# Icelk/strange-attractor-renderer

Measured on AMD Instinct MI355X. Metric: attractor iterations/sec at 1e9 iters, 2048x2048 buffer (poisson-saturne), per-GPU frame, higher is better.
Workload: dtype f64

## Files before the change

strange_attractor_renderer_amd/csrc/sar_iterate.hip:

```cpp
#include "sar_device.hpp"
#include "sar_launch.hpp"

namespace sar {

__global__ void __launch_bounds__(256) k_iterate(const IterArgs a) {
    const uint32_t job = blockIdx.x * blockDim.x + threadIdx.x;
    if (job >= a.n_jobs) return;
    MapParams p = a.p;
#pragma unroll
    for (int k = 0; k < 9; ++k) p.m[k] = vgpr_pin(p.m[k]);
    p.sin_v = vgpr_pin(p.sin_v);
    p.cos_v = vgpr_pin(p.cos_v);
    p.ccx = vgpr_pin(p.ccx);
    p.ccy = vgpr_pin(p.ccy);
    p.ccz = vgpr_pin(p.ccz);
    p.width = vgpr_pin(p.width);
    p.height = vgpr_pin(p.height);
    p.half_height = vgpr_pin(p.half_height);
    p.width_scaled = vgpr_pin(p.width_scaled);
    p.scale_adjusted_mid = vgpr_pin(p.scale_adjusted_mid);

    double x = a.starts[job];
    double y = a.starts[a.n_jobs + job];
    double z = a.starts[2u * a.n_jobs + job];

    if (!a.resume)
        for (int w = 0; w < 1000; ++w) next_point(p, x, y, z);

    const uint32_t n = (uint32_t)a.iters;
    const uint32_t lo_base = 0xFFFFFFFFu - job * n;
    const uint32_t C = a.ckpt_stride;
    const size_t cs = a.n_jobs;

    uint32_t t = 0;
    double* ck = a.ckpt + job;
    bool ended = false;
    while (t < n && !ended) {
        ck[0] = x;
        ck[cs] = y;
        ck[2 * cs] = z;
        ck += 3 * cs;
        const uint32_t tend = (n - t > C) ? t + C : n;
        for (; t < tend; ++t) {
            next_point(p, x, y, z);
            if (x != x) {
                __hip_atomic_fetch_add(a.scratch_count, n - t, __ATOMIC_RELAXED, __HIP_MEMORY_SCOPE_AGENT);
                ended = true;
                break;
            }
            double sx, sy, sz;
            screen_space(p, x, y, z, sx, sy, sz);
            const double ax = sx + p.ccx;
            const double az = sz + p.ccy;
            const double x2 = ax * p.cos_v + az * p.sin_v;
            const double z2 = ax * p.sin_v - az * p.cos_v;
            const double fi = (p.scale_adjusted_mid - x2) * p.width_scaled;
            const double fj = p.half_height - (sy + p.ccz) * p.width_scaled;
            if (fi >= p.width || fj >= p.height || fi < 0. || fj < 0.) continue;
            const uint32_t i = (fi == fi) ? (uint32_t)fi : 0u;
            const uint32_t j = (fj == fj) ? (uint32_t)fj : 0u;
            const uint32_t idx = j * a.width + i;
            __hip_atomic_fetch_add(a.scratch_count + idx, 1u, __ATOMIC_RELAXED, __HIP_MEMORY_SCOPE_AGENT);
            float zf = (float)z2;
            if (zf > -1.0f) {
                zf = zf + 0.0f;
                const unsigned long long k =
                    ((unsigned long long)f32_sortable(zf) << 32) | (unsigned long long)(lo_base - t);
                __hip_atomic_fetch_max(a.scratch_key + idx, k, __ATOMIC_RELAXED, __HIP_MEMORY_SCOPE_AGENT);
            }
        }
    }
    if (a.state_out) {
        a.state_out[job] = x;
        a.state_out[a.n_jobs + job] = y;
        a.state_out[2u * a.n_jobs + job] = z;
    }
}


template <bool DEPTH, uint32_t U, typename H, uint32_t W = 0>
struct DepthPipe {
    static_assert(W % U == 0, "a park window is whole passes of the depth pipeline");
    static constexpr bool kWide = sizeof(H) == 4;
    H* zhint;
    unsigned long long* key;
    uint32_t lo_base;
    HintQuant hq;
    HintTile ht;
    bool pv[U];
    uint32_t p_idx[U], p_zf[U], p_hint[U], p_q[U], n_sent, n_pass;
    uint32_t p_t[U];
    bool gv[U];
    uint32_t g_idx[U], g_q[U];
    unsigned long long g_mine[U], g_cur[U];
    unsigned long long q_m;
    unsigned long long pvm[U];
    uint32_t q_idx, q_zf, q_t;

    __device__ __forceinline__ uint32_t hint_index(uint32_t idx) const {
        if (kWide) return idx;
        return bfi(ht.mask2, bfi(ht.mask1, idx >> ht.shift1, idx << 3), idx);
    }
    __device__ __forceinline__ void depth_init(H* zhint_, unsigned long long* key_, uint32_t lo_base_, const uint32_t* hint_range_, const HintTile& tile_) {
        ht = tile_;
        zhint = zhint_;
        key = key_;
        lo_base = lo_base_;
        hq = hint_quant(kWide ? nullptr : hint_range_);
        n_sent = n_pass = 0;
#pragma unroll
        for (uint32_t k = 0; k < U; ++k) {
            pv[k] = gv[k] = false;
            p_idx[k] = p_zf[k] = p_hint[k] = p_q[k] = p_t[k] = 0;
            g_idx[k] = g_q[k] = 0;
            g_mine[k] = g_cur[k] = 0;
        }
        q_m = 0ull;
#pragma unroll
        for (uint32_t k = 0; k < U; ++k) pvm[k] = 0ull;
        q_idx = q_zf = q_t = 0;
    }

#ifdef SAR_EXPERIMENT_PROF
    unsigned long long dprof[2] = {0, 0};
#define SAR_DMARK(i, t0) do { asm volatile("s_waitcnt vmcnt(0)" ::: "memory"); const unsigned long long n_ = __builtin_readcyclecounter(); dprof[i] += n_ - t0; t0 = n_; } while (0)
#else
#define SAR_DMARK(i, t0)
#endif
    __device__ __forceinline__ void key_settle(uint32_t k) {
        if (g_mine[k] > g_cur[k]) {
            atomicMax(key + g_idx[k], g_mine[k]);
            ++n_sent;
        }
        const uint32_t seen = (uint32_t)(g_cur[k] >> 32);
        uint32_t learnt;
        if (kWide) {
            const float mine = __uint_as_float(g_q[k]), theirs = sortable_f32(seen);
            learnt = (seen && theirs > mine) ? __float_as_uint(theirs) : g_q[k];
        } else {
            const uint32_t qs = seen ? depth_q16(sortable_f32(seen), hq) : 0u;
            learnt = qs > g_q[k] ? qs : g_q[k];
        }
        zhint[hint_index(g_idx[k])] = (H)learnt;
    }
    __device__ __forceinline__ void key_request(uint32_t k, uint32_t idx, uint32_t zf, uint32_t q, uint32_t t) {
        ++n_pass;
        const float zc = __uint_as_float(zf) + 0.0f;
        g_idx[k] = idx;
        g_q[k] = kWide ? __float_as_uint(zc) : q;
        g_mine[k] = ((unsigned long long)f32_sortable(zc) << 32) | (unsigned long long)(lo_base - t);
        g_cur[k] = __hip_atomic_load(key + idx, __ATOMIC_RELAXED, __HIP_MEMORY_SCOPE_AGENT);
    }
    __device__ __forceinline__ bool hint_passed(uint32_t k) const {
        if (kWide) return pv[k] && __uint_as_float(p_zf[k]) >= __uint_as_float(p_hint[k]);
        const uint32_t hint = (p_idx[k] & 1u) ? (p_hint[k] >> 16) : (p_hint[k] & 0xFFFFu);
        return pv[k] && p_q[k] >= hint;
    }
    __device__ __forceinline__ void settle_depth(uint32_t k) {
#ifdef SAR_EXPERIMENT_PROF
        unsigned long long t0_ = __builtin_readcyclecounter();
#endif
        if (gv[k]) key_settle(k);
        SAR_DMARK(0, t0_);
        gv[k] = hint_passed(k);
        if (gv[k]) key_request(k, p_idx[k], p_zf[k], p_q[k], p_t[k]);
        SAR_DMARK(1, t0_);
    }

    __device__ __forceinline__ unsigned long long pass_mask(uint32_t k) const {
        if (kWide) return pvm[k] & __builtin_amdgcn_fcmpf(__uint_as_float(p_zf[k]), __uint_as_float(p_hint[k]), 3 );
        const uint32_t hint = (p_idx[k] & 1u) ? (p_hint[k] >> 16) : (p_hint[k] & 0xFFFFu);
        return pvm[k] & lanes_ge(p_q[k], hint);
    }
    __device__ __forceinline__ void park_flush() {
        if (gv[0]) key_settle(0);
        const bool parked = __builtin_amdgcn_inverse_ballot_w64(q_m);
        gv[0] = parked;
        if (parked) key_request(0, q_idx, q_zf, kWide ? 0u : depth_q16(__uint_as_float(q_zf) + 0.0f, hq), q_t);
        q_m = 0ull;
    }
    __device__ __forceinline__ void settle_parked(uint32_t k, bool window) {
        const unsigned long long pm = pass_mask(k);
        if (window || (pm & q_m) != 0ull) park_flush();
        q_m |= pm;
        if (__builtin_amdgcn_inverse_ballot_w64(pm)) {
            q_idx = p_idx[k];
            q_zf = p_zf[k];
            q_t = p_t[k];
            asm volatile("" : "+v"(q_idx), "+v"(q_zf), "+v"(q_t));
        }
    }

    __device__ __forceinline__ bool depth_candidate(uint32_t k, bool inb, uint32_t idx, float zf, uint32_t t) {
        if (!DEPTH) return false;
        if (W) settle_parked(k, k == 0u && (t & (W - 1u)) == 0u);
        else settle_depth(k);
        p_idx[k] = idx;
        p_zf[k] = __float_as_uint(zf);
        p_t[k] = t;
        if (kWide) {
            pv[k] = inb;
            if (W) pvm[k] = wave_ballot(inb);
            return inb;
        }
        const bool cand = inb && zf > -1.0f;
        p_q[k] = depth_q16(zf + 0.0f, hq);
        pv[k] = cand;
        if (W) pvm[k] = wave_ballot(inb) & __builtin_amdgcn_fcmpf(zf, -1.0f, 2 );
        return cand;
    }

    __device__ __forceinline__ void depth_request(uint32_t k, bool cand, uint32_t idx) {
        if (DEPTH) p_hint[k] = *(const uint32_t*)(zhint + (cand ? (kWide ? idx : (hint_index(idx) & ~1u)) : 0u));
    }

    __device__ __forceinline__ void depth_drain(uint32_t lane, unsigned long long* stats) {
        if (!DEPTH) return;
        if (W) {
#pragma unroll
            for (uint32_t k = 0; k < U; ++k) {
                settle_parked(k, false);
                pv[k] = false;
                pvm[k] = 0ull;
            }
            park_flush();
            park_flush();
        } else {
#pragma unroll
            for (uint32_t k = 0; k < U; ++k) {
                settle_depth(k);
                pv[k] = false;
            }
#pragma unroll
            for (uint32_t k = 0; k < U; ++k) settle_depth(k);
        }
        uint32_t tot = n_sent, pas = n_pass;
        for (int off = 32; off > 0; off >>= 1) {
            tot += __shfl_down(tot, off);
            pas += __shfl_down(pas, off);
        }
        if (lane == 0 && tot) atomicAdd(stats + 1, (unsigned long long)tot);
        if (lane == 0 && pas) atomicAdd(stats + 14, (unsigned long long)pas);
    }
};

template <bool DEPTH, uint32_t R, uint32_t U, typename H, uint32_t W = 0>
struct PoolStager : DepthPipe<DEPTH, U, H, W> {
    using DepthPipe<DEPTH, U, H, W>::depth_init;
    using DepthPipe<DEPTH, U, H, W>::depth_candidate;
    using DepthPipe<DEPTH, U, H, W>::depth_request;
    using DepthPipe<DEPTH, U, H, W>::depth_drain;
    static constexpr uint32_t CB = kPoolChunkBytes(R);
    static constexpr uint32_t Q = CB / 16u;
    static constexpr uint32_t P = kPoolSpareOf(R);
    static constexpr uint32_t kFillBits = 7u, kFillMask = 127u;
    uint32_t* ctl;
    uint32_t* ring;
    uint32_t pool0;
    uint32_t lane, n_bins;
    uint4* arena;
    uint32_t cursor;
    uint32_t drained;
    BinMap map;
    uint32_t bin_bits_v;
    bool b_have;
    uint32_t b_bin, b_old, b_local;
#ifdef SAR_EXPERIMENT_PROF
    unsigned long long prof[8] = {0, 0, 0, 0, 0, 0, 0, 0}, prof_last = 0;
    __device__ __forceinline__ void mark(int i) {
        asm volatile("" ::: "memory");
        const unsigned long long now = __builtin_readcyclecounter();
        asm volatile("" ::: "memory");
        prof[i] += now - prof_last;
        prof_last = now;
    }
#define SAR_MARK(i) this->mark(i)
#else
#define SAR_MARK(i)
#endif

    static __device__ __forceinline__ uint32_t lds_addr(const void* p) { return (uint32_t)(uintptr_t)(const __attribute__((address_space(3))) void*)p; }
    static __device__ __forceinline__ char* lds_ptr(uint32_t a) { return (char*)(__attribute__((address_space(3))) char*)(uintptr_t)a; }

    __device__ __forceinline__ void init(char* wbase, uint32_t bins, uint32_t lane_, uint4* arena_, H* zhint_,
                                         unsigned long long* key_, const BinMap& map_, uint32_t lo_base_, const uint32_t* hint_range_, const HintTile& tile_) {
        n_bins = bins;
        lane = lane_;
        char* pool = wbase;
        ctl = (uint32_t*)(wbase + (bins + P) * CB);
        ring = ctl + bins;
        pool0 = lds_addr(pool) + 8u;
        for (uint32_t b = lane; b < bins; b += 64u) {
            ctl[b] = (pool0 + b * CB) << kFillBits;
            *(uint2*)(pool + b * CB) = make_uint2(kNoChunk, R);
        }
        if (lane < P) ring[lane] = pool0 + (bins + lane) * CB;
        arena = arena_;
        cursor = drained = 0;
        depth_init(zhint_, key_, lo_base_, hint_range_, tile_);
        map = map_;
        bin_bits_v = map_.bin_bits;
        asm volatile("" : "+v"(bin_bits_v));
        b_have = false;
        b_bin = b_old = b_local = 0;
    }

    __device__ __forceinline__ void drain_all() {
        constexpr uint32_t G = kChunkLanes(R);
        static_assert(P <= 64u / G, "one pass must cover the ring");
        const uint32_t q = lane % G;
        const uint32_t e = drained + lane / G;
        if ((int32_t)(cursor - e) > 0 && q < Q) {
            const uint32_t rec = ring[e % P];
            const u32x4 v = *(const u32x4*)lds_ptr(rec - 8u + q * 16u);
            __builtin_nontemporal_store(v, (u32x4*)(arena + (size_t)e * kChunkStride(R)) + q);
        }
        drained = cursor;
    }

    __device__ __forceinline__ void swap_round(bool mine, uint32_t rank, uint32_t count, uint32_t bin, uint32_t rec) {
        if (cursor - drained + count > P) drain_all();
        if (mine) {
            const uint32_t chunk = cursor + rank;
            const uint32_t fresh = __hip_atomic_exchange(&ring[chunk % P], rec, __ATOMIC_RELAXED, __HIP_MEMORY_SCOPE_WORKGROUP);
            *(uint2*)lds_ptr(fresh - 8u) = make_uint2(chunk, R);
            __hip_atomic_fetch_add(&ctl[bin], ((fresh - rec) << kFillBits) - R, __ATOMIC_RELAXED, __HIP_MEMORY_SCOPE_WORKGROUP);
        }
        cursor = __builtin_amdgcn_readfirstlane(cursor + count);
    }
    __device__ __forceinline__ void swap_full(bool fl, unsigned long long fb, uint32_t bin, uint32_t rec) {
        const uint32_t rank = __builtin_amdgcn_mbcnt_hi((uint32_t)(fb >> 32), __builtin_amdgcn_mbcnt_lo((uint32_t)fb, 0u));
        const uint32_t nfill = (uint32_t)__popcll(fb);
        if (nfill <= P) {
            swap_round(fl, rank, nfill, bin, rec);
        } else {
            for (uint32_t base = 0; base < nfill; base += P)
                swap_round(fl && rank - base < P, rank - base, nfill - base < P ? nfill - base : P, bin, rec);
        }
    }

    __device__ __forceinline__ void place_visit() {
        uint32_t slot = b_old & kFillMask;
        uint32_t rec = b_old >> kFillBits;
        const bool w0 = b_have && slot < R;
        if (w0) *(unsigned short*)lds_ptr(rec + 2u * slot) = (unsigned short)b_local;
        const unsigned long long fb = lanes_eq(slot, R - 1u) & wave_ballot(b_have);
        const bool fl = b_have && slot == R - 1u;
        if (fb) {
            swap_full(fl, fb, b_bin, rec);
            if (__builtin_expect(lanes_ge(b_have ? slot : 0u, R) != 0ull, 0)) place_overflow(slot, rec);
        }
    }
    __device__ __forceinline__ void place_overflow(uint32_t slot, uint32_t rec) {
        bool over = b_have && slot >= R;
        for (;;) {
            slot -= over ? R : 0u;
            if (over) rec = ctl[b_bin] >> kFillBits;
            const bool w = over && slot < R;
            if (w) *(unsigned short*)lds_ptr(rec + 2u * slot) = (unsigned short)b_local;
            const bool fl = w && slot == R - 1u;
            over = over && slot >= R;
            const unsigned long long fb = wave_ballot(fl);
            if (!fb) break;
            swap_full(fl, fb, b_bin, rec);
            if (!wave_ballot(over)) break;
        }
    }

    __device__ __forceinline__ void step(uint32_t k, bool inb, uint32_t idx, float zf, uint32_t t) {
        __builtin_amdgcn_s_setprio(3);
        place_visit();
        SAR_MARK(2);
        const bool cand = depth_candidate(k, inb, idx, zf, t);
        SAR_MARK(3);
        b_have = inb;
        b_bin = __builtin_amdgcn_ubfe(idx, map.seg_shift, bin_bits_v);
        b_local = bfi(map.low_mask, idx, idx >> map.hi_shift);
        if (inb) b_old = atomicAdd(&ctl[b_bin], 1u);
        depth_request(k, cand, idx);
        __builtin_amdgcn_s_setprio(0);
        SAR_MARK(4);
    }

    __device__ __forceinline__ void finish(uint32_t* heads, uint32_t n_waves, uint32_t wave, unsigned long long* stats) {
        place_visit();
        drain_all();
        depth_drain(lane, stats);
        for (uint32_t b0 = 0; b0 < n_bins; b0 += 64u) {
            const uint32_t b = b0 + lane;
            const uint32_t word = (b < n_bins) ? ctl[b] : (pool0 << kFillBits);
            const uint32_t have = (b < n_bins) ? (word & kFillMask) : 0u;
            const bool flusher = have != 0u;
            const unsigned long long fb = wave_ballot(flusher);
            const uint32_t rec = word >> kFillBits;
            uint32_t head = (b < n_bins) ? *(const uint32_t*)lds_ptr(rec - 8u) : kNoChunk;
            if (flusher) {
                const uint32_t chunk = cursor + __builtin_amdgcn_mbcnt_hi((uint32_t)(fb >> 32),
                                                                          __builtin_amdgcn_mbcnt_lo((uint32_t)fb, 0u));
                *(uint32_t*)lds_ptr(rec - 4u) = have;
                u32x4* dst = (u32x4*)(arena + (size_t)chunk * kChunkStride(R));
#pragma unroll
                for (uint32_t q = 0; q < Q; ++q)
                    __builtin_nontemporal_store(*(const u32x4*)lds_ptr(rec - 8u + q * 16u), dst + q);
                head = chunk;
            }
            cursor += (uint32_t)__popcll(fb);
            if (b < n_bins) heads[(size_t)b * n_waves + wave] = head;
        }
    }
};

constexpr int kWarmupRangeIters = 64;
__device__ __forceinline__ void warmup_body(const WarmArgs& a) {
    const double* __restrict__ starts = a.starts;
    double* __restrict__ warm = a.warm;
    uint32_t* __restrict__ joblist = a.joblist;
    uint32_t* const hint_range = a.hint_range;
    const uint32_t n_jobs = a.n_jobs;
    const uint32_t slot_in = blockIdx.x * blockDim.x + threadIdx.x;
    const uint32_t n_in = a.in_active ? *a.in_active : n_jobs;
    if (blockIdx.x * blockDim.x >= n_in) return;
    const bool valid = slot_in < n_in;
    const uint32_t job = (valid && a.in_joblist) ? a.in_joblist[slot_in] : slot_in;
    const int n_iter = (int)a.n_iter;
    MapParams p = a.p;
    pin_map_params(p);
    double x = 0., y = 0., z = 0.;
    float zlo = __builtin_inff(), zhi = -__builtin_inff();
    if (valid) {
        x = starts[slot_in];
        y = starts[n_jobs + slot_in];
        z = starts[2u * n_jobs + slot_in];
        if (!hint_range) {
            for (int w = 0; w < n_iter; ++w) next_point(p, x, y, z);
        } else {
            const int n_range = n_iter < kWarmupRangeIters ? n_iter : kWarmupRangeIters;
            for (int w = 0; w < n_iter - n_range; ++w) next_point(p, x, y, z);
            for (int w = 0; w < n_range; ++w) {
                bool inb;
                uint32_t idx;
                float zf;
                iterate_once(p, a.width, x, y, z, inb, idx, zf);
                if (inb && zf > -1.0f) {
                    zlo = fminf(zlo, zf);
                    zhi = fmaxf(zhi, zf);
                }
            }
        }
    }
    if (hint_range) {
        for (int off = 32; off > 0; off >>= 1) {
            zlo = fminf(zlo, __shfl_down(zlo, off));
            zhi = fmaxf(zhi, __shfl_down(zhi, off));
        }
        if ((threadIdx.x & 63u) == 0u && zhi >= zlo) {
            atomicMax(hint_range, ~f32_sortable(zlo + 0.0f));
            atomicMax(hint_range + 1, f32_sortable(zhi + 0.0f));
        }
    }
    const bool live = valid && x == x;
    const unsigned long long lm = wave_ballot(live), dm = wave_ballot(valid && !live);
    const uint32_t rank = __builtin_amdgcn_mbcnt_hi((uint32_t)(lm >> 32), __builtin_amdgcn_mbcnt_lo((uint32_t)lm, 0u));
    uint32_t base = 0;
    if ((threadIdx.x & 63u) == 0u) {
        if (lm) base = atomicAdd(a.active, (uint32_t)__popcll(lm));
        if (dm) atomicAdd(a.nan_count, a.iters * (unsigned long long)__popcll(dm));
    }
    base = __builtin_amdgcn_readfirstlane(base);
    if (live) {
        const uint32_t slot = base + rank;
        warm[slot] = x;
        warm[n_jobs + slot] = y;
        warm[2u * n_jobs + slot] = z;
        joblist[slot] = job;
    }
}
__global__ void __launch_bounds__(256) k_warmup(const WarmArgs a) { warmup_body(a); }

__global__ void __launch_bounds__(256) k_warmup_batch(const BatchFrame* frames, uint32_t first_phase) {
    const WarmArgs a = load_frame_args(first_phase ? &frames[blockIdx.z].warm_first : &frames[blockIdx.z].warm);
    warmup_body(a);
}
__global__ void __launch_bounds__(256) k_batch_clear(const BatchFrame* frames) {
    const BatchFrame* f = frames + blockIdx.y;
    uint32_t* const seg = f->seg_any;
    const uint32_t n = f->seg_words;
    for (uint32_t k = blockIdx.x * blockDim.x + threadIdx.x; k < n; k += gridDim.x * blockDim.x) seg[k] = 0u;
    if (blockIdx.x == 0u && threadIdx.x < 4u) f->warm.active[threadIdx.x] = 0u;
    if (blockIdx.x == 0u && threadIdx.x < 4u && f->warm_first.n_iter) f->warm_first.active[threadIdx.x] = 0u;
    if (blockIdx.x == 0u && threadIdx.x < 2u && f->clear_hint_range) f->warm.hint_range[threadIdx.x] = 0u;
}

template <bool DEPTH, uint32_t R, uint32_t U, typename H>
__global__ void __launch_bounds__(256) k_iterate_lean(const BinIterArgs a) {
    extern __shared__ __attribute__((aligned(16))) uint32_t smem[];
    const uint32_t lane = threadIdx.x & 63u;
    const uint32_t slot = blockIdx.x * blockDim.x + threadIdx.x;
    const uint32_t wave = slot >> 6;
    const uint32_t active = *a.active;
    if (a.warm_nan && slot == 0u) {
        const unsigned long long dead = *a.warm_nan;
        if (dead) atomicAdd(a.nan_count, dead);
    }
    if ((slot & ~63u) >= active) {
        for (uint32_t b = lane; b < a.n_bins; b += 64u) a.heads[(size_t)b * a.n_waves + wave] = kNoChunk;
        return;
    }
    bool alive = slot < active;
    const uint32_t job = alive ? a.joblist[slot] : 0u;
    const uint32_t n = (uint32_t)a.it.iters;

    PoolStager<DEPTH, R, U, H> st;
    st.init((char*)smem + (threadIdx.x >> 6) * kPoolWaveLds(a.n_bins, R), a.n_bins, lane,
            (uint4*)a.arena + (size_t)wave * a.chunks_per_wave * kChunkStride(R),
            (H*)a.zhint + (size_t)(xcc_id() & a.hint_copy_mask) * kHintStride(a.it.npix), a.it.scratch_key, a.map, 0xFFFFFFFFu - job * n, a.hint_range, a.tile);

    MapParams p = a.it.p;
    pin_map_params(p);
#pragma unroll
    for (int k = 0; k < 10; ++k) p.cy[k] = vgpr_pin(p.cy[k]);
    double x = 0., y = 0., z = 0.;
    if (alive) {
        x = a.warm[slot];
        y = a.warm[a.it.n_jobs + slot];
        z = a.warm[2u * a.it.n_jobs + slot];
    }
    const uint32_t C = a.it.ckpt_stride;
    const size_t cs = a.it.n_jobs;
    uint32_t t = 0;
    double* ck = a.it.ckpt + job;
    auto checkpoint = [&]() {
        {
            const bool ended = alive && x != x;
            if (wave_ballot(ended)) {
                if (ended) atomicAdd(a.nan_count, (unsigned long long)(n - t));
                alive = alive && !ended;
            }
        }
        if (alive) {
            __builtin_nontemporal_store(x, ck);
            __builtin_nontemporal_store(y, ck + cs);
            __builtin_nontemporal_store(z, ck + 2 * cs);
        }
        ck += 3 * cs;
    };
    auto iteration = [&](uint32_t k) {
        bool inb;
        uint32_t idx;
        float zf;
        iterate_once(p, a.it.width, x, y, z, inb, idx, zf);
        inb = inb && alive;
#ifdef SAR_EXPERIMENT_PROF
        asm volatile("" : "+v"(idx), "+v"(zf));
#endif
#ifdef SAR_EXPERIMENT_PROF
        st.mark(0);
#endif
        st.step(k, inb, idx, zf, t);
        ++t;
    };
#ifdef SAR_EXPERIMENT_PROF
    st.prof_last = __builtin_readcyclecounter();
#endif
    const uint32_t n_full = n - n % U;
    while (t < n_full) {
        checkpoint();
        const uint32_t tend = (n_full - t > C) ? t + C : n_full;
        while (t < tend) {
#pragma unroll
            for (uint32_t k = 0; k < U; ++k) iteration(k);
        }
    }
    if (t < n) {
        if (t % C == 0u) checkpoint();
#pragma unroll
        for (uint32_t k = 0; k + 1 < U; ++k)
            if (t < n) iteration(k);
    }
#ifdef SAR_EXPERIMENT_PROF
    if (lane == 0)
        for (int i = 0; i < 4; ++i) atomicAdd(a.nan_count + 2 + i, st.prof[i ? i + 1 : i]);
#endif
    if (a.warm_out && slot < active) {
        a.warm_out[slot] = x;
        a.warm_out[a.it.n_jobs + slot] = y;
        a.warm_out[2u * a.it.n_jobs + slot] = z;
    }
    st.finish(a.heads, a.n_waves, wave, a.nan_count);
}

template <bool DEPTH, uint32_t R, uint32_t U, typename H, uint32_t PH, uint32_t W = 0>
__device__ __forceinline__ void iterate_split_body(const BinIterArgs& a, uint32_t* smem, const uint32_t wave) {
    static_assert(PH == 1u || PH == U, "a phase is one iteration or one pass of the depth pipeline");
    const uint32_t lane = threadIdx.x & 63u;
    const bool producer = threadIdx.x < 64u;
    const uint32_t slot = wave * 64u + lane;
    const uint32_t active = *a.active;
    if (a.warm_nan && wave == 0u && threadIdx.x == 0u) {
        const unsigned long long dead = *a.warm_nan;
        if (dead) atomicAdd(a.nan_count, dead);
    }
    if (wave * 64u >= active) {
        if (!producer)
            for (uint32_t b = lane; b < a.n_bins; b += 64u) a.heads[(size_t)b * a.n_waves + wave] = kNoChunk;
        return;
    }
    bool alive = slot < active;
    const uint32_t job = alive ? a.joblist[slot] : 0u;
    const uint32_t n = (uint32_t)a.it.iters;
    uint2* hand = (uint2*)((char*)smem + kPoolWaveLds(a.n_bins, R));
    const uint32_t n_full = n - n % U;
    if (producer) {
        MapParams p = a.it.p;
        pin_map_params(p);
#pragma unroll
        for (int k = 0; k < 10; ++k) p.cy[k] = vgpr_pin(p.cy[k]);
        double x = 0., y = 0., z = 0.;
        if (alive) {
            x = a.warm[slot];
            y = a.warm[a.it.n_jobs + slot];
            z = a.warm[2u * a.it.n_jobs + slot];
        }
        const uint32_t C = a.it.ckpt_stride;
        const size_t cs = a.it.n_jobs;
        double* ck = a.it.ckpt + job;
        uint32_t t = 0;
        auto checkpoint = [&]() {
            const bool ended = alive && x != x;
            if (wave_ballot(ended)) {
                if (ended) atomicAdd(a.nan_count, (unsigned long long)(n - t));
                alive = alive && !ended;
            }
            if (alive) {
                __builtin_nontemporal_store(x, ck);
                __builtin_nontemporal_store(y, ck + cs);
                __builtin_nontemporal_store(z, ck + 2 * cs);
            }
            ck += 3 * cs;
        };
        auto produce = [&](uint2* dst) {
            bool inb;
            uint32_t idx;
            float zf;
            iterate_once(p, a.it.width, x, y, z, inb, idx, zf);
            inb = inb && alive;
            *dst = make_uint2(inb ? idx : 0xFFFFFFFFu, __float_as_uint(zf));
            ++t;
        };
        uint32_t phase = 0;
#ifdef SAR_EXPERIMENT_PROF
        unsigned long long pp[2] = {0, 0}, pl = __builtin_readcyclecounter();
#define SAR_PMARK(i) do { asm volatile("" ::: "memory"); const unsigned long long now_ = __builtin_readcyclecounter(); asm volatile("" ::: "memory"); pp[i] += now_ - pl; pl = now_; } while (0)
#else
#define SAR_PMARK(i)
#endif
        while (t < n_full) {
            checkpoint();
            const uint32_t tend = (n_full - t > C) ? t + C : n_full;
            while (t < tend) {
#pragma unroll
                for (uint32_t h = 0; h < U / PH; ++h) {
                    uint2* dst = hand + (phase & 1u) * (PH * 64u) + lane;
#pragma unroll
                    for (uint32_t k = 0; k < PH; ++k) produce(dst + k * 64u);
                    asm volatile("s_waitcnt lgkmcnt(0)" ::: "memory");
                    SAR_PMARK(0);
                    asm volatile("s_barrier" ::: "memory");
                    SAR_PMARK(1);
                    ++phase;
                }
            }
        }
#ifdef SAR_EXPERIMENT_PROF
        if (lane == 0) { atomicAdd(a.nan_count + 6, pp[0]); atomicAdd(a.nan_count + 7, pp[1]); }
#endif
        if (t < n) {
            if (t % C == 0u) checkpoint();
#pragma unroll
            for (uint32_t k = 0; k + 1 < U; ++k)
                if (t < n) {
                    produce(hand + (phase & 1u) * (PH * 64u) + lane);
                    asm volatile("s_waitcnt lgkmcnt(0)\n\ts_barrier" ::: "memory");
                    ++phase;
                }
        }
        if (a.warm_out && slot < active) {
            a.warm_out[slot] = x;
            a.warm_out[a.it.n_jobs + slot] = y;
            a.warm_out[2u * a.it.n_jobs + slot] = z;
        }
    } else {
        PoolStager<DEPTH, R, U, H, W> st;
        st.init((char*)smem, a.n_bins, lane, (uint4*)a.arena + (size_t)wave * a.chunks_per_wave * kChunkStride(R),
                (H*)a.zhint + (size_t)(xcc_id() & a.hint_copy_mask) * kHintStride(a.it.npix), a.it.scratch_key, a.map, 0xFFFFFFFFu - job * n, a.hint_range, a.tile);
        uint32_t t = 0, phase = 0;
#ifdef SAR_EXPERIMENT_PROF
        st.prof_last = __builtin_readcyclecounter();
#endif
        while (t < n_full) {
#pragma unroll
            for (uint32_t h = 0; h < U / PH; ++h) {
                asm volatile("s_barrier" ::: "memory");
#ifdef SAR_EXPERIMENT_PROF
                st.mark(0);
#endif
                const uint2* src = hand + (phase & 1u) * (PH * 64u) + lane;
                uint2 v[PH];
#pragma unroll
                for (uint32_t k = 0; k < PH; ++k) v[k] = src[k * 64u];
#ifdef SAR_EXPERIMENT_PROF
#pragma unroll
                for (uint32_t k = 0; k < PH; ++k) asm volatile("" : "+v"(v[k].x), "+v"(v[k].y));
                st.mark(1);
#endif
#pragma unroll
                for (uint32_t k = 0; k < PH; ++k) {
                    st.step(h * PH + k, v[k].x != 0xFFFFFFFFu, v[k].x, __uint_as_float(v[k].y), t);
                    ++t;
                }
                ++phase;
            }
        }
#pragma unroll
        for (uint32_t k = 0; k + 1 < U; ++k)
            if (t < n) {
                asm volatile("s_barrier" ::: "memory");
                const uint2 v = hand[(phase & 1u) * (PH * 64u) + lane];
                st.step(k, v.x != 0xFFFFFFFFu, v.x, __uint_as_float(v.y), t);
                ++t;
                ++phase;
            }
#ifdef SAR_EXPERIMENT_PROF
        if (lane == 0) {
            for (int i = 0; i < 5; ++i) atomicAdd(a.nan_count + 8 + i, st.prof[i]);
            atomicAdd(a.nan_count + 13, st.dprof[0]);
            atomicAdd(a.nan_count + 15, st.dprof[1]);
        }
#endif
        st.finish(a.heads, a.n_waves, wave, a.nan_count);
    }
}
template <bool DEPTH, uint32_t R, uint32_t U, typename H, uint32_t PH, uint32_t W>
__global__ void __launch_bounds__(128) k_iterate_split(const BinIterArgs a) {
    extern __shared__ __attribute__((aligned(16))) uint32_t smem[];
    iterate_split_body<DEPTH, R, U, H, PH, W>(a, smem, blockIdx.x);
}
template <bool DEPTH, uint32_t R, uint32_t U, typename H, uint32_t PH>
__global__ void __launch_bounds__(128) k_iterate_split_batch(const BatchFrame* frames, uint32_t n_frames, uint32_t n_waves, uint32_t xcd_map) {
    extern __shared__ __attribute__((aligned(16))) uint32_t smem[];
    const uint32_t lin = blockIdx.x;
    uint32_t frame, wave;
    if (xcd_map == 1u) {
        const uint32_t xpf = 8u / n_frames, xcd = lin & 7u, pos = lin >> 3;
        frame = xcd / xpf;
        wave = pos * xpf + xcd % xpf;
    } else if (xcd_map == 2u) {
        const uint32_t xcd = lin & 7u, pos = lin >> 3, turn = pos / n_waves;
        frame = xcd + 8u * turn;
        wave = pos - turn * n_waves;
    } else if (xcd_map == 3u) {
        const uint32_t total = n_frames * n_waves, xcd = lin & 7u, pos = lin >> 3;
        const uint32_t q = total >> 3, r = total & 7u;
        const uint32_t g = xcd * q + (xcd < r ? xcd : r) + pos;
        frame = g / n_waves;
        wave = g - frame * n_waves;
    } else {
        frame = lin / n_waves;
        wave = lin - frame * n_waves;
    }
    const BinIterArgs a = load_frame_args(&frames[frame].it);
    iterate_split_body<DEPTH, R, U, H, PH>(a, smem, wave);
}

__device__ __forceinline__ void bound(double v, double& lo, double& hi) {
    lo = v < lo ? v : lo;
    hi = v > hi ? v : hi;
}

__global__ void __launch_bounds__(256) k_extent(const MapParams pin, const double* __restrict__ starts, uint32_t n_jobs,
                                                uint64_t iters, double* __restrict__ out) {
    __shared__ double part[4][12];
    const uint32_t job = blockIdx.x * blockDim.x + threadIdx.x;
    MapParams p = pin;
    pin_map_params(p);
    double b[12];
#pragma unroll
    for (int k = 0; k < 6; ++k) {
        b[2 * k] = __builtin_inf();
        b[2 * k + 1] = -__builtin_inf();
    }
    if (job < n_jobs) {
        double x = starts[job], y = starts[n_jobs + job], z = starts[2u * n_jobs + job];
        for (int w = 0; w < 1000; ++w) next_point(p, x, y, z);
        for (uint64_t t = 0; t < iters; ++t) {
            next_point(p, x, y, z);
            double sx, sy, sz;
            screen_space(p, x, y, z, sx, sy, sz);
            bound(sx, b[0], b[1]);
            bound(sy, b[2], b[3]);
            bound(sz, b[4], b[5]);
            bound(x, b[6], b[7]);
            bound(y, b[8], b[9]);
            bound(z, b[10], b[11]);
        }
    }
#pragma unroll
    for (int k = 0; k < 12; ++k) {
        double v = b[k];
        for (int off = 32; off > 0; off >>= 1) {
            const double o = __shfl_down(v, off);
            v = (k & 1) ? (o > v ? o : v) : (o < v ? o : v);
        }
        if ((threadIdx.x & 63u) == 0) part[threadIdx.x >> 6][k] = v;
    }
    __syncthreads();
    if (threadIdx.x < 12) {
        const int k = threadIdx.x;
        double v = part[0][k];
        for (uint32_t w = 1; w < blockDim.x / 64u; ++w) {
            const double o = part[w][k];
            v = (k & 1) ? (o > v ? o : v) : (o < v ? o : v);
        }
        out[(size_t)blockIdx.x * 12u + k] = v;
    }
}

__global__ void __launch_bounds__(256) k_starts_soa(const double* __restrict__ aos, double* __restrict__ soa, uint32_t m) {
    const uint32_t k = blockIdx.x * blockDim.x + threadIdx.x;
    if (k < m) {
        soa[k] = aos[3u * k];
        soa[m + k] = aos[3u * k + 1u];
        soa[2u * m + k] = aos[3u * k + 2u];
    }
}

void launch_iterate(const IterArgs& a, uint32_t block, hipStream_t s) {
    hipLaunchKernelGGL(k_iterate, dim3((a.n_jobs + block - 1) / block), dim3(block), 0, s, a);
}

uint32_t lean_wave_lds_bytes(uint32_t bins, uint32_t records) { return kPoolWaveLds(bins, records); }
uint32_t chunk_bytes(uint32_t records) { return kChunkStride(records) * 16u; }

#define SAR_FOR_EACH_LEAN(X)                                                                                         \
    X(12u, unsigned short) X(20u, unsigned short) X(28u, unsigned short) X(60u, unsigned short)                       \
    X(12u, uint32_t) X(20u, uint32_t) X(28u, uint32_t) X(60u, uint32_t)
#define SAR_FOR_EACH_SPLIT(X)                                                                                        \
    X(28u, unsigned short, 1u) X(28u, unsigned short, 2u) X(28u, uint32_t, 1u) X(28u, uint32_t, 2u)                   \
    X(60u, unsigned short, 1u) X(60u, unsigned short, 2u) X(60u, uint32_t, 1u) X(60u, uint32_t, 2u)

#define SAR_FOR_EACH_PARK(X, RR, HH, PP) X(RR, HH, PP, 0u) X(RR, HH, PP, 2u) X(RR, HH, PP, 4u) X(RR, HH, PP, 8u)

int launch_iterate_lean(const BinIterArgs& a, uint32_t block, uint32_t records, uint32_t hint_bytes, bool split, uint32_t park, hipStream_t s) {
    const uint32_t stage = lean_wave_lds_bytes(a.n_bins, records);
    bool launched = false;
    if (split) {
        const uint32_t ph = (stage + 2048u) * 8u <= 160u * 1024u ? 2u : 1u;
        const size_t lds2 = stage + ph * 1024u;
#define SAR_LAUNCH_PARK(RR, HH, PP, WW)                                                                               \
    if (!launched && records == RR && hint_bytes == sizeof(HH) && ph == PP && park == WW) {                            \
        hipLaunchKernelGGL((k_iterate_split<true, RR, 2u, HH, PP, WW>), dim3(a.n_waves), dim3(128), lds2, s, a);       \
        launched = true;                                                                                              \
    }
#define SAR_LAUNCH_SPLIT(RR, HH, PP) SAR_FOR_EACH_PARK(SAR_LAUNCH_PARK, RR, HH, PP)
        SAR_FOR_EACH_SPLIT(SAR_LAUNCH_SPLIT)
#undef SAR_LAUNCH_SPLIT
#undef SAR_LAUNCH_PARK
        return launched ? 0 : 1;
    }
    if (park) return 1;
    const uint32_t grid = (a.it.n_jobs + block - 1) / block;
    const size_t lds = (size_t)(block / 64u) * stage;
#define SAR_LAUNCH_LEAN(RR, HH)                                                                                       \
    if (!launched && records == RR && hint_bytes == sizeof(HH)) {                                                      \
        hipLaunchKernelGGL((k_iterate_lean<true, RR, 2u, HH>), dim3(grid), dim3(block), lds, s, a);                    \
        launched = true;                                                                                              \
    }
    SAR_FOR_EACH_LEAN(SAR_LAUNCH_LEAN)
#undef SAR_LAUNCH_LEAN
    return launched ? 0 : 1;
}

uint32_t batch_xcd_map(uint32_t n_frames, uint32_t n_waves) {
    if (n_frames <= 8u && 8u % n_frames == 0u && n_waves % (8u / n_frames) == 0u) return 1;
    if (n_frames % 8u == 0u) return 2;
    if (n_frames >= 3u) return 3;
    return 0;
}

int launch_iterate_split_batch(const BatchFrame* frames, uint32_t n_frames, uint32_t n_waves, uint32_t n_bins, uint32_t records,
                               uint32_t hint_bytes, uint32_t xcd_map, hipStream_t s) {
    const uint32_t total = n_frames * n_waves;
    const uint32_t stage = lean_wave_lds_bytes(n_bins, records);
    const uint32_t ph = (stage + 2048u) * 8u <= 160u * 1024u ? 2u : 1u;
    const size_t lds2 = stage + ph * 1024u;
    bool launched = false;
#define SAR_LAUNCH_SPLIT_BATCH(RR, HH, PP)                                                                                        \
    if (!launched && records == RR && hint_bytes == sizeof(HH) && ph == PP) {                                                      \
        hipLaunchKernelGGL((k_iterate_split_batch<true, RR, 2u, HH, PP>), dim3(total), dim3(128), lds2, s, frames, n_frames, n_waves, xcd_map); \
        launched = true;                                                                                                          \
    }
    SAR_FOR_EACH_SPLIT(SAR_LAUNCH_SPLIT_BATCH)
#undef SAR_LAUNCH_SPLIT_BATCH
    return launched ? 0 : 1;
}

int iterate_kernel_attributes() {
    hipError_t e = hipSuccess;
#define SAR_ATTR_LEAN(RR, HH) \
    if (e == hipSuccess) e = hipFuncSetAttribute((const void*)k_iterate_lean<true, RR, 2u, HH>, hipFuncAttributeMaxDynamicSharedMemorySize, 160 * 1024);
    SAR_FOR_EACH_LEAN(SAR_ATTR_LEAN)
#undef SAR_ATTR_LEAN
#define SAR_ATTR_PARK(RR, HH, PP, WW) \
    if (e == hipSuccess) e = hipFuncSetAttribute((const void*)k_iterate_split<true, RR, 2u, HH, PP, WW>, hipFuncAttributeMaxDynamicSharedMemorySize, 160 * 1024);
#define SAR_ATTR_SPLIT(RR, HH, PP) SAR_FOR_EACH_PARK(SAR_ATTR_PARK, RR, HH, PP)
    SAR_FOR_EACH_SPLIT(SAR_ATTR_SPLIT)
#undef SAR_ATTR_SPLIT
#undef SAR_ATTR_PARK
#define SAR_ATTR_SPLIT_BATCH(RR, HH, PP) \
    if (e == hipSuccess) e = hipFuncSetAttribute((const void*)k_iterate_split_batch<true, RR, 2u, HH, PP>, hipFuncAttributeMaxDynamicSharedMemorySize, 160 * 1024);
    SAR_FOR_EACH_SPLIT(SAR_ATTR_SPLIT_BATCH)
#undef SAR_ATTR_SPLIT_BATCH
    return (int)e;
}

uint32_t launch_extent(const MapParams& p, const double* starts, uint32_t n_jobs, uint64_t iters, double* out, hipStream_t s) {
    const uint32_t blocks = (n_jobs + 255u) / 256u;
    hipLaunchKernelGGL(k_extent, dim3(blocks), dim3(256), 0, s, p, starts, n_jobs, iters, out);
    return blocks;
}

void launch_starts_soa(const double* aos, double* soa, uint32_t m, hipStream_t s) {
    hipLaunchKernelGGL(k_starts_soa, dim3((m + 255u) / 256u), dim3(256), 0, s, aos, soa, m);
}

__global__ void k_dead_jobs(const uint32_t* active, uint32_t n_jobs, uint64_t iters, unsigned long long* nan_count) {
    const uint32_t dead = n_jobs - *active;
    if (dead) atomicAdd(nan_count, iters * (unsigned long long)dead);
}
void launch_dead_jobs(const uint32_t* active, uint32_t n_jobs, uint64_t iters, unsigned long long* nan_count, hipStream_t s) {
    hipLaunchKernelGGL(k_dead_jobs, dim3(1), dim3(1), 0, s, active, n_jobs, iters, nan_count);
}

void launch_warmup(const WarmArgs& a, hipStream_t s) {
    hipLaunchKernelGGL(k_warmup, dim3((a.n_jobs + 255u) / 256u), dim3(256), 0, s, a);
}
void launch_warmup_batch(const BatchFrame* frames, uint32_t n_frames, uint32_t n_jobs, bool first_phase, hipStream_t s) {
    hipLaunchKernelGGL(k_warmup_batch, dim3((n_jobs + 255u) / 256u, 1, n_frames), dim3(256), 0, s, frames, first_phase ? 1u : 0u);
}
__global__ void __launch_bounds__(256) k_batch_fetch(const BatchFrame* frames) {
    const BatchFrame* f = frames + blockIdx.y;
    const u32x4* __restrict__ src = (const u32x4*)f->starts_host;
    u32x4* __restrict__ dst = (u32x4*)f->starts_dev;
    const uint32_t n = f->n_start_quads;
    for (uint32_t k = blockIdx.x * blockDim.x + threadIdx.x; k < n; k += gridDim.x * blockDim.x) dst[k] = src[k];
}
void launch_batch_fetch(const BatchFrame* frames, uint32_t n_frames, hipStream_t s) {
    hipLaunchKernelGGL(k_batch_fetch, dim3(32, n_frames), dim3(256), 0, s, frames);
}
void launch_batch_clear(const BatchFrame* frames, uint32_t n_frames, uint32_t seg_words, hipStream_t s) {
    hipLaunchKernelGGL(k_batch_clear, dim3((seg_words + 255u) / 256u, n_frames), dim3(256), 0, s, frames);
}

}
```

Before: 170.8 billion.

## Flag off-screen visits in the pixel index and reuse a per-step lane mask

Producers now mark a missing visit by setting the top bit of the pixel index, so consumer waves form the visit mask with one vector compare and reuse it for slot writes, full-chunk detection and depth parking, where several ballots were computed before. The per-bin control word is kept as a precomputed LDS address. The wide depth-hint load skips its select by relying on the flagged index staying in range. The consumer loop is unrolled over paired hand-over halves so the phase parity becomes a compile-time constant. This adds template machinery and depends on the flagged index offset staying inside the hint buffer.

```diff
diff --git a/strange_attractor_renderer_amd/csrc/sar_iterate.hip b/strange_attractor_renderer_amd/csrc/sar_iterate.hip
--- a/strange_attractor_renderer_amd/csrc/sar_iterate.hip
+++ b/strange_attractor_renderer_amd/csrc/sar_iterate.hip
@@ -78,6 +78,22 @@
 }
 
 
+struct PlainVisit {
+    static constexpr bool kFlagged = false;
+    uint32_t idx;
+    bool inb;
+    __device__ __forceinline__ unsigned long long lanes() const { return wave_ballot(inb); }
+    __device__ __forceinline__ bool here(unsigned long long) const { return inb; }
+};
+constexpr uint32_t kNoVisit = 0x80000000u;
+static_assert((unsigned long long)kMaxBins * kMaxBinPx <= (1ull << 30), "a pixel index of the binned path times four must fit 32 bits");
+struct FlaggedVisit {
+    static constexpr bool kFlagged = true;
+    uint32_t idx;
+    __device__ __forceinline__ unsigned long long lanes() const { return __builtin_amdgcn_uicmp(idx, kNoVisit, 36 ); }
+    __device__ __forceinline__ bool here(unsigned long long m) const { return __builtin_amdgcn_inverse_ballot_w64(m); }
+};
+
 template <bool DEPTH, uint32_t U, typename H, uint32_t W = 0>
 struct DepthPipe {
     static_assert(W % U == 0, "a park window is whole passes of the depth pipeline");
@@ -191,7 +207,7 @@
         }
     }
 
-    __device__ __forceinline__ bool depth_candidate(uint32_t k, bool inb, uint32_t idx, float zf, uint32_t t) {
+    __device__ __forceinline__ bool depth_candidate(uint32_t k, bool inb, unsigned long long have, uint32_t idx, float zf, uint32_t t) {
         if (!DEPTH) return false;
         if (W) settle_parked(k, k == 0u && (t & (W - 1u)) == 0u);
         else settle_depth(k);
@@ -200,18 +216,21 @@
         p_t[k] = t;
         if (kWide) {
             pv[k] = inb;
-            if (W) pvm[k] = wave_ballot(inb);
+            if (W) pvm[k] = have;
             return inb;
         }
         const bool cand = inb && zf > -1.0f;
         p_q[k] = depth_q16(zf + 0.0f, hq);
         pv[k] = cand;
-        if (W) pvm[k] = wave_ballot(inb) & __builtin_amdgcn_fcmpf(zf, -1.0f, 2 );
+        if (W) pvm[k] = have & __builtin_amdgcn_fcmpf(zf, -1.0f, 2 );
         return cand;
     }
 
+    template <bool FLAGGED>
     __device__ __forceinline__ void depth_request(uint32_t k, bool cand, uint32_t idx) {
-        if (DEPTH) p_hint[k] = *(const uint32_t*)(zhint + (cand ? (kWide ? idx : (hint_index(idx) & ~1u)) : 0u));
+        if (!DEPTH) return;
+        if (FLAGGED && kWide) p_hint[k] = *(const uint32_t*)((const char*)zhint + (size_t)(uint32_t)(idx << 2));
+        else p_hint[k] = *(const uint32_t*)(zhint + (cand ? (kWide ? idx : (hint_index(idx) & ~1u)) : 0u));
     }
 
     __device__ __forceinline__ void depth_drain(uint32_t lane, unsigned long long* stats) {
@@ -248,7 +267,6 @@
 struct PoolStager : DepthPipe<DEPTH, U, H, W> {
     using DepthPipe<DEPTH, U, H, W>::depth_init;
     using DepthPipe<DEPTH, U, H, W>::depth_candidate;
-    using DepthPipe<DEPTH, U, H, W>::depth_request;
     using DepthPipe<DEPTH, U, H, W>::depth_drain;
     static constexpr uint32_t CB = kPoolChunkBytes(R);
     static constexpr uint32_t Q = CB / 16u;
@@ -263,8 +281,8 @@
     uint32_t drained;
     BinMap map;
     uint32_t bin_bits_v;
-    bool b_have;
-    uint32_t b_bin, b_old, b_local;
+    unsigned long long b_have;
+    uint32_t b_ctl, b_old, b_local;
 #ifdef SAR_EXPERIMENT_PROF
     unsigned long long prof[8] = {0, 0, 0, 0, 0, 0, 0, 0}, prof_last = 0;
     __device__ __forceinline__ void mark(int i) {
@@ -301,8 +319,8 @@
         map = map_;
         bin_bits_v = map_.bin_bits;
         asm volatile("" : "+v"(bin_bits_v));
-        b_have = false;
-        b_bin = b_old = b_local = 0;
+        b_have = 0ull;
+        b_ctl = b_old = b_local = 0;
     }
 
     __device__ __forceinline__ void drain_all() {
@@ -318,66 +336,70 @@
         drained = cursor;
     }
 
-    __device__ __forceinline__ void swap_round(bool mine, uint32_t rank, uint32_t count, uint32_t bin, uint32_t rec) {
+    __device__ __forceinline__ void swap_round(bool mine, uint32_t rank, uint32_t count, uint32_t ctl_a, uint32_t rec) {
         if (cursor - drained + count > P) drain_all();
         if (mine) {
             const uint32_t chunk = cursor + rank;
             const uint32_t fresh = __hip_atomic_exchange(&ring[chunk % P], rec, __ATOMIC_RELAXED, __HIP_MEMORY_SCOPE_WORKGROUP);
             *(uint2*)lds_ptr(fresh - 8u) = make_uint2(chunk, R);
-            __hip_atomic_fetch_add(&ctl[bin], ((fresh - rec) << kFillBits) - R, __ATOMIC_RELAXED, __HIP_MEMORY_SCOPE_WORKGROUP);
+            __hip_atomic_fetch_add((uint32_t*)lds_ptr(ctl_a), ((fresh - rec) << kFillBits) - R, __ATOMIC_RELAXED, __HIP_MEMORY_SCOPE_WORKGROUP);
         }
         cursor = __builtin_amdgcn_readfirstlane(cursor + count);
     }
-    __device__ __forceinline__ void swap_full(bool fl, unsigned long long fb, uint32_t bin, uint32_t rec) {
+    __device__ __forceinline__ void swap_full(bool fl, unsigned long long fb, uint32_t ctl_a, uint32_t rec) {
         const uint32_t rank = __builtin_amdgcn_mbcnt_hi((uint32_t)(fb >> 32), __builtin_amdgcn_mbcnt_lo((uint32_t)fb, 0u));
         const uint32_t nfill = (uint32_t)__popcll(fb);
         if (nfill <= P) {
-            swap_round(fl, rank, nfill, bin, rec);
+            swap_round(fl, rank, nfill, ctl_a, rec);
         } else {
             for (uint32_t base = 0; base < nfill; base += P)
-                swap_round(fl && rank - base < P, rank - base, nfill - base < P ? nfill - base : P, bin, rec);
+                swap_round(fl && rank - base < P, rank - base, nfill - base < P ? nfill - base : P, ctl_a, rec);
         }
     }
 
     __device__ __forceinline__ void place_visit() {
-        uint32_t slot = b_old & kFillMask;
-        uint32_t rec = b_old >> kFillBits;
-        const bool w0 = b_have && slot < R;
-        if (w0) *(unsigned short*)lds_ptr(rec + 2u * slot) = (unsigned short)b_local;
-        const unsigned long long fb = lanes_eq(slot, R - 1u) & wave_ballot(b_have);
-        const bool fl = b_have && slot == R - 1u;
+        const uint32_t slot = b_old & kFillMask;
+        const uint32_t rec = b_old >> kFillBits;
+        if (__builtin_amdgcn_inverse_ballot_w64(b_have & ~lanes_ge(slot, R))) *(unsigned short*)lds_ptr(rec + 2u * slot) = (unsigned short)b_local;
+        const unsigned long long fb = lanes_eq(slot, R - 1u) & b_have;
         if (fb) {
-            swap_full(fl, fb, b_bin, rec);
-            if (__builtin_expect(lanes_ge(b_have ? slot : 0u, R) != 0ull, 0)) place_overflow(slot, rec);
-        }
-    }
-    __device__ __forceinline__ void place_overflow(uint32_t slot, uint32_t rec) {
-        bool over = b_have && slot >= R;
+            swap_full(__builtin_amdgcn_inverse_ballot_w64(fb), fb, b_ctl, rec);
+            const unsigned long long ob = lanes_ge(slot, R) & b_have;
+            if (__builtin_expect(ob != 0ull, 0)) place_overflow(ob, slot, rec);
+        }
+    }
+    __device__ __forceinline__ void place_overflow(unsigned long long ob, uint32_t slot, uint32_t rec) {
+        bool over = __builtin_amdgcn_inverse_ballot_w64(ob);
         for (;;) {
             slot -= over ? R : 0u;
-            if (over) rec = ctl[b_bin] >> kFillBits;
+            if (over) rec = *(const uint32_t*)lds_ptr(b_ctl) >> kFillBits;
             const bool w = over && slot < R;
             if (w) *(unsigned short*)lds_ptr(rec + 2u * slot) = (unsigned short)b_local;
             const bool fl = w && slot == R - 1u;
             over = over && slot >= R;
             const unsigned long long fb = wave_ballot(fl);
             if (!fb) break;
-            swap_full(fl, fb, b_bin, rec);
+            swap_full(fl, fb, b_ctl, rec);
             if (!wave_ballot(over)) break;
         }
     }
 
-    __device__ __forceinline__ void step(uint32_t k, bool inb, uint32_t idx, float zf, uint32_t t) {
+    template <typename V>
+    __device__ __forceinline__ void step(uint32_t k, const V& v, float zf, uint32_t t) {
         __builtin_amdgcn_s_setprio(3);
         place_visit();
         SAR_MARK(2);
-        const bool cand = depth_candidate(k, inb, idx, zf, t);
+        const uint32_t idx = v.idx;
+        const unsigned long long have = v.lanes();
+        const bool inb = v.here(have);
+        const bool cand = depth_candidate(k, inb, have, idx, zf, t);
         SAR_MARK(3);
-        b_have = inb;
-        b_bin = __builtin_amdgcn_ubfe(idx, map.seg_shift, bin_bits_v);
+        b_have = have;
+        b_ctl = lds_addr(ctl) + 4u * __builtin_amdgcn_ubfe(idx, map.seg_shift, bin_bits_v);
+        asm volatile("" : "+v"(b_ctl));
         b_local = bfi(map.low_mask, idx, idx >> map.hi_shift);
-        if (inb) b_old = atomicAdd(&ctl[b_bin], 1u);
-        depth_request(k, cand, idx);
+        if (inb) b_old = atomicAdd((uint32_t*)lds_ptr(b_ctl), 1u);
+        this->template depth_request<V::kFlagged>(k, cand, idx);
         __builtin_amdgcn_s_setprio(0);
         SAR_MARK(4);
     }
@@ -556,7 +578,7 @@
 #ifdef SAR_EXPERIMENT_PROF
         st.mark(0);
 #endif
-        st.step(k, inb, idx, zf, t);
+        st.step(k, PlainVisit{idx, inb}, zf, t);
         ++t;
     };
 #ifdef SAR_EXPERIMENT_PROF
@@ -644,7 +666,7 @@
             float zf;
             iterate_once(p, a.it.width, x, y, z, inb, idx, zf);
             inb = inb && alive;
-            *dst = make_uint2(inb ? idx : 0xFFFFFFFFu, __float_as_uint(zf));
+            *dst = make_uint2(inb ? idx : kNoVisit, __float_as_uint(zf));
             ++t;
         };
         uint32_t phase = 0;
@@ -697,36 +719,43 @@
 #ifdef SAR_EXPERIMENT_PROF
         st.prof_last = __builtin_readcyclecounter();
 #endif
-        while (t < n_full) {
-#pragma unroll
-            for (uint32_t h = 0; h < U / PH; ++h) {
-                asm volatile("s_barrier" ::: "memory");
-#ifdef SAR_EXPERIMENT_PROF
-                st.mark(0);
-#endif
-                const uint2* src = hand + (phase & 1u) * (PH * 64u) + lane;
-                uint2 v[PH];
-#pragma unroll
-                for (uint32_t k = 0; k < PH; ++k) v[k] = src[k * 64u];
-#ifdef SAR_EXPERIMENT_PROF
-#pragma unroll
-                for (uint32_t k = 0; k < PH; ++k) asm volatile("" : "+v"(v[k].x), "+v"(v[k].y));
-                st.mark(1);
-#endif
-#pragma unroll
-                for (uint32_t k = 0; k < PH; ++k) {
-                    st.step(h * PH + k, v[k].x != 0xFFFFFFFFu, v[k].x, __uint_as_float(v[k].y), t);
-                    ++t;
-                }
-                ++phase;
-            }
+        auto run_phase = [&](uint32_t k0, uint32_t half) {
+            asm volatile("s_barrier" ::: "memory");
+#ifdef SAR_EXPERIMENT_PROF
+            st.mark(0);
+#endif
+            const uint2* src = hand + half * (PH * 64u) + lane;
+            uint2 v[PH];
+#pragma unroll
+            for (uint32_t k = 0; k < PH; ++k) v[k] = src[k * 64u];
+#ifdef SAR_EXPERIMENT_PROF
+#pragma unroll
+            for (uint32_t k = 0; k < PH; ++k) asm volatile("" : "+v"(v[k].x), "+v"(v[k].y));
+            st.mark(1);
+#endif
+#pragma unroll
+            for (uint32_t k = 0; k < PH; ++k) {
+                st.step(k0 + k, FlaggedVisit{v[k].x}, __uint_as_float(v[k].y), t);
+                ++t;
+            }
+            ++phase;
+        };
+        constexpr uint32_t kTripPhases = U / PH > 2u ? U / PH : 2u, kTripSteps = kTripPhases * PH;
+        static_assert(kTripPhases % 2u == 0u && kTripSteps % U == 0u, "a trip starts on half 0 of the hand-over and slot 0 of the pipeline");
+        while (n_full - t >= kTripSteps) {
+#pragma unroll
+            for (uint32_t h = 0; h < kTripPhases; ++h) run_phase(h * PH % U, h & 1u);
+        }
+        if (kTripSteps > U && t < n_full) {
+#pragma unroll
+            for (uint32_t h = 0; h < U / PH; ++h) run_phase(h * PH, h & 1u);
         }
 #pragma unroll
         for (uint32_t k = 0; k + 1 < U; ++k)
             if (t < n) {
                 asm volatile("s_barrier" ::: "memory");
                 const uint2 v = hand[(phase & 1u) * (PH * 64u) + lane];
-                st.step(k, v.x != 0xFFFFFFFFu, v.x, __uint_as_float(v.y), t);
+                st.step(k, FlaggedVisit{v.x}, __uint_as_float(v.y), t);
                 ++t;
                 ++phase;
             }
```

Result: faster. 174.7 billion, median of 6 (+2.3%).
